# dguilliams3/book-recommendation-engine

Hardware: AMD Instinct MI355X
Metric: exact top-10 queries/sec at 10M×1536 fp32 (1/8 GPU) + % HBM/MFMA roofline (higher is better)
Workload: dtype fp32

## Files before the change

book-recommendation-engine_amd/csrc/vs_gemm_x1.hip:

```cpp
#include <algorithm>
#include <climits>
#include <cmath>
#include <cstdlib>
#include <type_traits>
#include <vector>

#include "vs_x1_device.h"

#ifndef VS_X1_PROBE
#define VS_X1_PROBE 0
#endif
#define VS_X1_P(bit) ((VS_X1_PROBE & (bit)) != 0)

namespace vs {

#ifndef VS_X1_STAMP
#define VS_X1_STAMP 0
#endif
constexpr int kStampSeg = 9;
constexpr int kStampCnt = 3;
constexpr int kStampHist = 16;
constexpr int kStampN = 2 * (kStampSeg + kStampCnt) + 2 + 2 * kStampHist;
__device__ unsigned long long g_x1_stamps[kStampN];

// ... 766 lines not shown
    auto seg_step = [&](auto first_tag) {
      constexpr bool first = decltype(first_tag)::value;
      __builtin_amdgcn_sched_barrier(0);
      if constexpr (S16) {
        rd16(buf);
      } else {
        rd(buf, 0, fa0, fb0);
        rd(buf, 1, fa1, fb1);
      }
      __builtin_amdgcn_sched_barrier(0);
      stage_step();
      advance_cursor();
      __builtin_amdgcn_sched_barrier(0);
      VS_X1_MARK(0);
      asm volatile("s_waitcnt vmcnt(8)" ::: "memory");
      VS_X1_MARK(1);
      __builtin_amdgcn_s_barrier();
      __builtin_amdgcn_sched_barrier(0);
      VS_X1_MARK(2);
      if constexpr (S16) {
#pragma unroll
        for (int b = 0; b < 8; ++b) mfma16_b(b, first_tag);
      } else {
        if constexpr (first) {
#pragma unroll
          for (int rb = 0; rb < 4; ++rb) mfma_rb_first(rb, fa0, fb0);
        } else {
#pragma unroll
          for (int rb = 0; rb < 4; ++rb) mfma_rb(rb, fa0, fb0);
        }
#pragma unroll
        for (int rb = 0; rb < 4; ++rb) mfma_rb(rb, fa1, fb1);
      }
      __builtin_amdgcn_sched_barrier(0);
      VS_X1_MARK(3);
      __builtin_amdgcn_s_barrier();
      __builtin_amdgcn_sched_barrier(0);
      VS_X1_MARK(4);
      VS_X1_MARK(5);
      buf = buf + 1 == NBUF ? 0 : buf + 1;
    };
    auto seg_tiles = [&]() {
      for (int t = t0; t < t1; ++t) {
        seg_step(std::true_type{});
        for (int k = 1; k < nksteps; ++k) seg_step(std::false_type{});
        if constexpr (!VS_X1_P(8)) {
          if constexpr (S16) epilogue16(t);
          else epilogue(t);
        } else if constexpr (S16) {
#pragma unroll
          for (int b = 0; b < 8; ++b)
#pragma unroll
            for (int qb = 0; qb < 4; ++qb) asm volatile("" ::"v"(acc16[b][qb]));
        } else {
#pragma unroll
          for (int rb = 0; rb < 4; ++rb)
#pragma unroll
            for (int qb = 0; qb < 2; ++qb) asm volatile("" ::"v"(acc[rb][qb]));
        }
        VS_X1_MARK(5);
      }
    };
    seg_tiles();
    if (!lag) __builtin_amdgcn_s_barrier();
#undef VS_X1_MARK
    }
#if VS_X1_STAMP
    {
      const int grp = w >= 4 ? 1 : 0;
      if (lane == 0) {
#pragma unroll
        for (int i = 0; i < kStampSeg; ++i)
          atomicAdd(&g_x1_stamps[grp * (kStampSeg + kStampCnt) + i], sg[i]);
        atomicAdd(&g_x1_stamps[2 * (kStampSeg + kStampCnt) + grp], (unsigned long long)nsteps);
      }
      if (lane == 0)
        atomicAdd(&g_x1_stamps[grp * (kStampSeg + kStampCnt) + kStampSeg], ecnt[0]);
      if constexpr (S16) {
        const int bin = nev < kStampHist ? nev : kStampHist - 1;
        for (int v = 0; v < kStampHist; ++v) {
          const unsigned long long m = __ballot(bin == v);
          if (lane == 0 && m)
            atomicAdd(&g_x1_stamps[2 * (kStampSeg + kStampCnt) + 2 + (chunk == 1 ? 0 : kStampHist) + v],
                      (unsigned long long)__popcll(m));
        }
      }
    }
#endif
    asm volatile("s_waitcnt vmcnt(0)" ::: "memory");
  }

  const int ln = (int)__builtin_amdgcn_mbcnt_hi(~0u, __builtin_amdgcn_mbcnt_lo(~0u, 0u));
  const int pl0 = sp * 4 + wr * 2 + (S16 ? (ln >> 4) & 1 : ln >> 5);
#pragma unroll
  for (int qb = 0; qb < NQB; ++qb) {
    const int64_t g =
        (int64_t)(qt * kT + 64 * wq + (S16 ? 16 * qb + (ln & 15) : 32 * qb + (ln & 31))) * P + pl0;
    if constexpr (VS_X1_P(256) && DUMP) {
      asm volatile("" ::"v"(dc[qb]), "v"(g));
    } else if constexpr (S16) {
      if (ln < 32) dcount[g] = dc[qb];
    } else if constexpr (DUMP) {
      dcount[g] = dc[qb];
    } else {
      const int64_t o = g * KP;
#pragma unroll
      for (int e = 0; e < KR; ++e) {
        pkey[o + e] = lk[qb][e];
        pid[o + e] = li[qb][e];
      }
      for (int e = KR; e < KP; ++e) {
        pkey[o + e] = FLT_MAX;
        pid[o + e] = -1;
      }
    }
  }
}

static int x1_qg() {
  static const int v = [] {
    const char* e = getenv("VS_X1_QG");
    const int q = e ? atoi(e) : 0;
    return q > 0 ? q : 4;
  }();
  return v;
}

static bool x1_group_rounds() {
  const char* e = getenv("VS_X1_XCDG");
  return !e || atoi(e) != 0;
}

constexpr int kX1SplitDen = 8;

constexpr int kX1ShortChunkTiles = 40;
static int x1_chunk_tiles(int per_block, bool can_dump) {
  const char* e = getenv("VS_X1_CHUNK_TILES");
  const int v = e ? atoi(e) : 0;
  if (v > 0) return v;
  return can_dump && per_block >= 128 && per_block <= 3 * kX1ChunkTiles ? kX1ShortChunkTiles
                                                                        : kX1ChunkTiles;
}

static int x1_split_den() {
  const char* e = getenv("VS_X1_SPLIT");
  return e ? std::max(0, atoi(e)) : kX1SplitDen;
}
constexpr int kSplitMinTiles = 16;
static int x1_first_den(int el, bool ecut) {
  const char* e = getenv("VS_X1_QUARTER");
  if (!e) return el == FILTER_BF16 || ecut ? 4 : 0;
  const int v = atoi(e);
  return v == 1 ? 4 : v >= 2 ? v : 0;
}

enum X1Kind : int { kX1List = 0, kX1Dump32 = 2, kX1Dump16 = 3 };
enum : int {
  kX1Replay = 1,
  kX1FirstCut = 2,
  kX1ReplayCut = 4,
  kX1ExactCut = 8,
};
struct X1Step {
  int p0, p1;
  int kind;
  int after;
};
struct X1Plan {
  int nparts = 1;
  bool cutting = false;
  std::vector<X1Step> step;
  int nlaunch() const { return (int)step.size(); }
};
static X1Plan x1_plan(int per_block, bool can_dump, int el, bool ecut, bool gathered, int recut) {
  X1Plan p;
  const bool dump = can_dump && !gathered;
  const int chunk_tiles = x1_chunk_tiles(per_block, dump);
  const int nchunk = gathered ? 1 : std::max(1, (per_block + chunk_tiles - 1) / chunk_tiles);
  const int den = x1_split_den();
  const bool split = dump && nchunk < 4 && den >= 2 && per_block >= kSplitMinTiles;
  p.cutting = dump && (nchunk >= 4 || split);
  const int F = x1_first_den(el, ecut);
  const bool quarter =
      p.cutting && !split && nchunk >= 4 && F >= 2 && per_block / (F * nchunk) >= 2;
  p.nparts = split ? den : quarter ? F * nchunk : nchunk;
  const int nlaunch = split ? 2 : quarter ? nchunk + 1 : nchunk;
  for (int c = 0; c < nlaunch; ++c) {
    X1Step s;
    s.p0 = split     ? (c == 0 ? 0 : 1)
           : quarter ? (c == 0 ? 0 : c == 1 ? 1 : F * (c - 1))
                     : c;
    s.p1 = split     ? (c == 0 ? 1 : den)
           : quarter ? (c == 0 ? 1 : F * c)
                     : c + 1;
    s.kind = p.cutting && c > 0 ? kX1Dump32 : kX1List;
    s.after = 0;
    if (p.cutting && c == 0) s.after |= kX1FirstCut | (ecut ? kX1ExactCut : 0);
    if (p.cutting && c > 0 && (((c + 1) & c) == 0 || c + 1 == nlaunch)) {
      const bool again = recut && c + 1 < nlaunch;
      s.after |= again ? kX1ReplayCut | (ecut ? kX1ExactCut : 0) : kX1Replay;
    }
    p.step.push_back(s);
  }
  return p;
}
static int x1_dump_kind(int mode, int el, bool dump32) {
  return x1_has_s16(mode, el) && !dump32 ? kX1Dump16 : kX1Dump32;
}

template <int KR, int MODE, int EL>
static hipError_t x1_launch(const X1Args& a, Partials part, hipStream_t st, int* ndispatch) {
  const int ntiles = (a.ntotal + kT - 1) / kT;
  const int nqt = a.nq_pad / kT;
  const int per_block = (ntiles + a.nsplit - 1) / a.nsplit;
  const int qg = a.qcount ? nqt : x1_qg() * (x1_group_rounds() ? 1 : -1);
  const bool dump = a.dump && x1_has_dump(MODE, EL) && !a.qcount && a.qcut && a.qbkey &&
                    a.qcut_m > 0 && a.dcount && a.dslot && a.dR > 0;
  const bool ecut = MODE == MODE_IP && EL == FILTER_I8 && a.ecut_x && a.qam;
  const X1Plan plan = x1_plan(per_block, dump, EL, ecut, a.qcount != nullptr, a.recut);
  const int nlaunch = plan.nlaunch();
  const int64_t ldb = a.ld * filter_bytes(EL);
  if (a.qtile0 < 0) return hipErrorInvalidValue;
  auto launch = [&](auto kernel, const X1Step& s, bool dumps) {
    hipLaunchKernelGGL(kernel, dim3(nqt * a.nsplit), dim3(512), 0, st, (const char*)a.XH, a.xs,
                       a.xaux, (const char*)a.QH, a.qs, a.qaux, a.nqa, (int)(ldb / 64), a.ntotal,
                       ntiles, a.nsplit, nqt, a.qtile0, a.self0, a.qrow, a.qcount, s.p0, s.p1,
                       plan.nparts, part.KP, qg, part.key, part.id, a.xgmax, a.xgmin,
                       dumps ? a.qcut : nullptr, dumps ? a.dcount : nullptr,
                       dumps ? a.dslot : nullptr, dumps ? a.dR : 0, a.qskip);
  };
  for (int c = 0; c < nlaunch; ++c) {
    const X1Step& s = plan.step[c];
    if (a.timing)
      a.timing->begin(st, !(plan.cutting && nlaunch > 1) || c > 0,
                      (double)(s.p1 - s.p0) / plan.nparts);
    switch (s.kind == kX1Dump32 ? x1_dump_kind(MODE, EL, a.dump32) : s.kind) {
      case kX1Dump16:
        if constexpr (x1_has_s16(MODE, EL))
          launch(gemm_topk_x1<KR, MODE, true, EL, true>, s, true);
        break;
      case kX1Dump32:
        if constexpr (x1_has_dump(MODE, EL)) launch(gemm_topk_x1<KR, MODE, true, EL>, s, true);
        break;
      default:
        launch(gemm_topk_x1<KR, MODE, false, EL>, s, false);
    }
    if (a.timing) a.timing->end(st);
    hipError_t e = hipGetLastError();
    if (e == hipSuccess && (s.after & kX1Replay)) e = launch_x1_replay(a, part, st);
    if (e == hipSuccess && (s.after & kX1FirstCut)) e = launch_qcut(a, part, st);
    if (e == hipSuccess && (s.after & kX1ReplayCut)) e = launch_x1_replay_cut(a, part, st);
    if (e == hipSuccess && (s.after & kX1ExactCut)) e = launch_x1_ecut(a, part, st);
    if (e != hipSuccess) return e;
  }
  if (ndispatch) *ndispatch = nlaunch;
  return hipSuccess;
}

int x1_lane_len() { return 8; }
int x1_dump_slots() { return kDumpMaxR; }
bool x1_pass_dumps(int ntotal, int nsplit) {
  const int ntiles = (ntotal + kT - 1) / kT;
  return x1_plan((ntiles + nsplit - 1) / nsplit, true, FILTER_I8, false, false, 1).cutting;
}

bool x1_plan_describe(int mode, int filter, int64_t ntotal, int nsplit, bool can_dump, bool ecut,
                      bool gathered, int recut, bool dump32, int32_t* out, int cap,
                      int* nlaunch) {
  if ((filter != FILTER_I8 && filter != FILTER_BF16) || ntotal <= 0 || ntotal > INT_MAX ||
      nsplit < 1 || (mode != MODE_IP && mode != MODE_L2 && mode != MODE_COS))
    return false;
  const int64_t ntiles = (ntotal + kT - 1) / kT;
  const X1Plan plan =
      x1_plan((int)((ntiles + nsplit - 1) / nsplit), can_dump && x1_has_dump(mode, filter), filter,
              ecut && mode == MODE_IP && filter == FILTER_I8, gathered, recut);
  out[0] = plan.nparts, out[1] = plan.cutting, out[2] = 0, out[3] = plan.cutting;
  out[4] = x1_pass_dumps((int)ntotal, nsplit);
  for (int c = 0; c < plan.nlaunch() && c < cap; ++c) {
    const X1Step& s = plan.step[c];
    int32_t* o = out + 5 + 4 * c;
    o[0] = s.p0, o[1] = s.p1, o[3] = s.after;
    o[2] = s.kind == kX1Dump32 ? x1_dump_kind(mode, filter, dump32) : s.kind;
  }
  *nlaunch = plan.nlaunch();
  return true;
}

hipError_t x1_stamps(unsigned long long* out, int reset) {
  hipError_t e = hipMemcpyFromSymbol(out, HIP_SYMBOL(g_x1_stamps), sizeof(g_x1_stamps));
  if (e == hipSuccess && reset) {
    unsigned long long z[kStampN] = {};
    e = hipMemcpyToSymbol(HIP_SYMBOL(g_x1_stamps), z, sizeof(z));
  }
  return e;
}

template <int EL>
static hipError_t x1_dispatch(int mode, const X1Args& a, Partials part, hipStream_t st,
                              int* ndispatch) {
  switch (mode) {
    case MODE_IP:
      return x1_launch<8, MODE_IP, EL>(a, part, st, ndispatch);
    case MODE_L2:
      if constexpr (EL == FILTER_I8) return hipErrorInvalidValue;
      else return x1_launch<8, MODE_L2, EL>(a, part, st, ndispatch);
    case MODE_COS:
      return x1_launch<8, MODE_COS, EL>(a, part, st, ndispatch);
    default:
      return hipErrorInvalidValue;
  }
}

hipError_t launch_gemm_topk_x1(int mode, const X1Args& a, Partials part, hipStream_t st,
                               int* ndispatch) {
  if (a.nq_pad % kT != 0 || a.ld % 64 != 0 || a.ld <= 0 || part.KP < x1_lane_len() ||
      part.P != 4 * a.nsplit || a.nsplit < 1 || a.ntotal <= 0)
    return hipErrorInvalidValue;
  if (a.filter == FILTER_I8) {
    if (!a.xs || !a.qs || !a.xgmax || !a.xgmin || a.ld > kI8MaxLd) return hipErrorInvalidValue;
    return x1_dispatch<FILTER_I8>(mode, a, part, st, ndispatch);
  }
  return x1_dispatch<FILTER_BF16>(mode, a, part, st, ndispatch);
}

bool x1_dump_applies(int mode, int filter) { return x1_has_dump(mode, filter); }

int x1_list_len(int need) {
  return need + 8 <= 24   ? 24
         : need + 8 <= 32 ? 32
         : need + 8 <= 64 ? 64
         : need < 128 ? 128
         : need < 256 ? 256
         : need < 512 ? 512
         : need < kVerifyMaxKF ? kVerifyMaxKF
                               : 0;
}

}
```

book-recommendation-engine_amd/csrc/vs_x1_cuts.hip:

```cpp
#include <algorithm>
#include <climits>
#include <cmath>
#include <cstdlib>

#include "vs_x1_device.h"

namespace vs {


template <int KR, int EL>
__global__ __launch_bounds__(256) void x1_replay_kernel(
    int* __restrict__ dcount, const int* __restrict__ dslot, float* __restrict__ pkey,
    int* __restrict__ pid, int P, int KP, int nqa, const float* __restrict__ qs,
    const float* __restrict__ xs, int64_t self0, int ntotal, int dR, int64_t nl,
    float* __restrict__ qcut, unsigned long long* __restrict__ stats) {
  const int64_t i = (int64_t)blockIdx.x * 256 + threadIdx.x;
  const int cnt = i < (int64_t)nqa * P ? dcount[i] : 0;
  replay_stats(cnt, dR, stats);
  if (cnt == 0) return;
  dcount[i] = 0;
  const int q = (int)(i / P);
  if (cnt > dR) {
    qcut[q] = -FLT_MAX;
    return;
  }
  const float cut = qcut[q];
  const float qsc = EL == FILTER_I8 ? qs[q] : 0.0f;
  const int selfrow = self0 >= 0 ? (int)(self0 + q) : -1;
  float lk[KR];
  int li[KR];
  const int64_t o = i * KP;
  lane_list_load<KR>(pkey, pid, o, lk, li);
  replay_admit<KR, EL>(lk, li, dslot, i, nl, cnt, qsc, xs, selfrow, ntotal, cut);
  lane_list_store<KR>(pkey, pid, o, lk, li);
}

hipError_t launch_x1_replay(const X1Args& a, Partials part, hipStream_t st) {
  unsigned long long* stats = a.dstats;
  if (!a.dump || !a.dcount || a.nqa <= 0) return hipSuccess;
  if (part.KP < x1_lane_len() || part.KP % 4 != 0) return hipErrorInvalidValue;
  const int64_t n = (int64_t)a.nqa * part.P;
  const dim3 grid((unsigned)((n + 255) / 256));
  const int64_t nl = (int64_t)a.nq_pad * part.P;
  if (a.filter == FILTER_I8)
    hipLaunchKernelGGL((x1_replay_kernel<8, FILTER_I8>), grid, dim3(256), 0, st, a.dcount, a.dslot,
                       part.key, part.id, part.P, part.KP, a.nqa, a.qs, a.xs, a.self0, a.ntotal,
                       a.dR, nl, a.qcut, stats);
  else
    hipLaunchKernelGGL((x1_replay_kernel<8, FILTER_BF16>), grid, dim3(256), 0, st, a.dcount,
                       a.dslot, part.key, part.id, part.P, part.KP, a.nqa, a.qs, a.xs, a.self0,
                       a.ntotal, a.dR, nl, a.qcut, stats);
  return hipGetLastError();
}

constexpr int kQcutThreads = 256;
__global__ __launch_bounds__(kQcutThreads) void qcut_kernel(
    const float* __restrict__ lkey, const int* __restrict__ lid, int P, int LKP, int L, int M,
    const double* __restrict__ bkey, int nq, float* __restrict__ cut, float* __restrict__ qam) {
  const int q = blockIdx.x;
  const int tid = threadIdx.x;
  if (q >= nq) return;
  const int64_t base = (int64_t)q * P * LKP;
  const int n = P * L;
  constexpr int kR = 16;
  uint64_t v[kR];
  const bool regs = n <= kQcutThreads * kR;
  auto image = [&](int j) -> uint64_t {
    const int64_t o = base + (int64_t)(j / L) * LKP + j % L;
    return lid[o] >= 0 ? (uint64_t)key_order(lkey[o]) : (1ull << 32);
  };
#pragma unroll
  for (int i = 0; i < kR; ++i) {
    const int j = tid + kQcutThreads * i;
    v[i] = regs && j < n ? image(j) : (1ull << 32);
  }
  __shared__ int part[kQcutThreads / 64];
  auto count_below = [&](uint64_t y) {
    int c = 0;
    if (regs) {
#pragma unroll
      for (int i = 0; i < kR; ++i) c += v[i] < y ? 1 : 0;
    } else {
      for (int j = tid; j < n; j += kQcutThreads) c += image(j) < y ? 1 : 0;
    }
    for (int o = 32; o > 0; o >>= 1) c += __shfl_xor(c, o);
    __syncthreads();
    if ((tid & 63) == 0) part[tid >> 6] = c;
    __syncthreads();
    int t = 0;
#pragma unroll
    for (int w = 0; w < kQcutThreads / 64; ++w) t += part[w];
    return t;
  };
  if (count_below(1ull << 32) < M) return;
  uint64_t x = 0;
  for (int b = 31; b >= 0; --b)
    if (count_below(x + (1ull << b)) < M) x += 1ull << b;
  const float aM = key_unorder((uint32_t)x);
  if (tid == 0 && qam) qam[q] = aM;
  if (tid == 0) {
    const float old = cut[q];
    const float t = lower_cut(aM, 2.000001, bkey[q], old);
    if (t < old) cut[q] = t;
  }
}

hipError_t launch_qcut(const X1Args& a, Partials part, hipStream_t st) {
  const int nq = a.nqa;
  hipLaunchKernelGGL(qcut_kernel, dim3(nq), dim3(kQcutThreads), 0, st, part.key, part.id, part.P, part.KP,
                     x1_lane_len(), a.qcut_m, a.qbkey, nq, a.qcut, a.qam);
  return hipGetLastError();
}

template <int KR, int EL>
__global__ __launch_bounds__(256) void x1_replay_cut_kernel(
    int* __restrict__ dcount, const int* __restrict__ dslot, float* __restrict__ pkey,
    int* __restrict__ pid, int P, int KP, const float* __restrict__ qs,
    const float* __restrict__ xs, int64_t self0, int ntotal, int dR, int64_t nl,
    float* __restrict__ qcut, unsigned long long* __restrict__ stats, int M,
    const double* __restrict__ bkey, float* __restrict__ qam) {
  __shared__ int hist[256];
  __shared__ int wsum[4];
  __shared__ int s_over, sel_digit, sel_before;
  const int q = blockIdx.x;
  const int tid = threadIdx.x, lane = tid & 63, wv = tid >> 6;
  const int nth = blockDim.x, nwv = nth >> 6;
  const bool has = tid < P;
  const int64_t i = (int64_t)q * P + tid;
  const int cnt = has ? dcount[i] : 0;
  replay_stats(cnt, dR, stats);
  if (tid == 0) s_over = 0;
  const float cut = qcut[q];
  float lk[KR];
  int li[KR];
  const int64_t o = i * KP;
#pragma unroll
  for (int e = 0; e < KR; ++e) lk[e] = FLT_MAX, li[e] = -1;
  if (has) lane_list_load<KR>(pkey, pid, o, lk, li);
  __syncthreads();
  if (cnt > 0) {
    dcount[i] = 0;
    if (cnt > dR) {
      s_over = 1;
    } else {
      const float qsc = EL == FILTER_I8 ? qs[q] : 0.0f;
      const int selfrow = self0 >= 0 ? (int)(self0 + q) : -1;
      replay_admit<KR, EL>(lk, li, dslot, i, nl, cnt, qsc, xs, selfrow, ntotal, cut);
      lane_list_store<KR>(pkey, pid, o, lk, li);
    }
  }
  __syncthreads();
  if (s_over) {
    if (tid == 0) qcut[q] = -FLT_MAX;
    return;
  }
  if (cut == -FLT_MAX) return;
  uint32_t v[KR];
  int nv = 0;
#pragma unroll
  for (int e = 0; e < KR; ++e) {
    v[e] = key_order(lk[e]);
    nv += li[e] >= 0 ? 1 : 0;
  }
  for (int o2 = 32; o2 > 0; o2 >>= 1) nv += __shfl_xor(nv, o2);
  if (lane == 0) wsum[wv] = nv;
  __syncthreads();
  int total = 0;
  for (int w2 = 0; w2 < nwv; ++w2) total += wsum[w2];
  if (total < M) return;
  uint32_t pre = 0;
  int want = M;
  for (int sh = 24; sh >= 0; sh -= 8) {
    for (int b = tid; b < 256; b += nth) hist[b] = 0;
    __syncthreads();
#pragma unroll
    for (int e = 0; e < KR; ++e)
      if (li[e] >= 0 && (sh == 24 || (v[e] >> (sh + 8)) == (pre >> (sh + 8))))
        atomicAdd(&hist[(v[e] >> sh) & 0xFF], 1);
    __syncthreads();
    if (wv == 0) {
      const int h0 = hist[4 * lane], h1 = hist[4 * lane + 1], h2 = hist[4 * lane + 2],
                h3 = hist[4 * lane + 3];
      const int own = h0 + h1 + h2 + h3;
      int inc = own;
      for (int o2 = 1; o2 < 64; o2 <<= 1) {
        const int t = __shfl_up(inc, o2);
        if (lane >= o2) inc += t;
      }
      const int before = inc - own;
      if (before < want && want <= inc) {
        int c = before, d = 4 * lane;
        const int hh[4] = {h0, h1, h2, h3};
        for (int e = 0; e < 4; ++e) {
          if (c + hh[e] >= want) {
            d = 4 * lane + e;
            break;
          }
          c += hh[e];
        }
        sel_digit = d;
        sel_before = c;
      }
    }
    __syncthreads();
    pre |= (uint32_t)sel_digit << sh;
    want -= sel_before;
  }
  if (tid == 0) {
    const float aM = key_unorder(pre);
    if (qam) qam[q] = aM;
    const float t = lower_cut(aM, 2.000001, bkey[q], cut);
    if (t < cut) qcut[q] = t;
  }
}

constexpr int kReplayCutMaxP = 256;

hipError_t launch_x1_replay_cut(const X1Args& a, Partials part, hipStream_t st) {
  if (!a.dump || !a.dcount || a.nqa <= 0) return hipSuccess;
  if (part.KP < x1_lane_len() || part.KP % 4 != 0) return hipErrorInvalidValue;
  if (a.recut == 2 || part.P > kReplayCutMaxP) {
    const hipError_t e = launch_x1_replay(a, part, st);
    return e != hipSuccess ? e : launch_qcut(a, part, st);
  }
  const int64_t nl = (int64_t)a.nq_pad * part.P;
  const dim3 block((unsigned)((part.P + 63) / 64 * 64));
  if (a.filter == FILTER_I8)
    hipLaunchKernelGGL((x1_replay_cut_kernel<8, FILTER_I8>), dim3(a.nqa), block, 0, st, a.dcount,
                       a.dslot, part.key, part.id, part.P, part.KP, a.qs, a.xs, a.self0, a.ntotal,
                       a.dR, nl, a.qcut, a.dstats, a.qcut_m, a.qbkey, a.qam);
  else
    hipLaunchKernelGGL((x1_replay_cut_kernel<8, FILTER_BF16>), dim3(a.nqa), block, 0, st, a.dcount,
                       a.dslot, part.key, part.id, part.P, part.KP, a.qs, a.xs, a.self0, a.ntotal,
                       a.dR, nl, a.qcut, a.dstats, a.qcut_m, a.qbkey, a.qam);
  return hipGetLastError();
}

constexpr int kEcutCand = 64;
__global__ __launch_bounds__(256) void x1_ecut_kernel(
    const float* __restrict__ lkey, const int* __restrict__ lid, int P, int LKP, int L, int M,
    const double* __restrict__ bkey, const float* __restrict__ qam, const float* __restrict__ X,
    const float* __restrict__ Q, int64_t ld, int ntotal, float* __restrict__ ckey,
    int* __restrict__ cid, float* __restrict__ qcut) {
  constexpr int kU = kEcutMaxM + kEcutCand;
  __shared__ int cand[kEcutCand];
  __shared__ float uk[kU];
  __shared__ int ui[kU];
  __shared__ int wsum[4];
  __shared__ int un;
  const int q = blockIdx.x;
  const int tid = threadIdx.x, lane = tid & 63, wv = tid >> 6;
  const float cut = qcut[q];
  const float aM = qam[q];
  float* ck = ckey + (int64_t)q * kEcutMaxM;
  int* ci = cid + (int64_t)q * kEcutMaxM;
  if (tid < kEcutMaxM) {
    ui[tid] = ci[tid];
    uk[tid] = ck[tid];
  }
  const float* qrow = Q + (int64_t)q * ld;
  const bool pairs = ld <= 256 * kQV;
  QSlice qsl;
  if (pairs) load_qslice(qrow, ld, lane, qsl);
  if (cut == -FLT_MAX || !(aM < FLT_MAX)) return;
  const bool vec = L == 8 && LKP % 4 == 0;
  int ncand = 0;
  for (int p0 = 0; p0 < P && ncand < kEcutCand; p0 += 256) {
    const int p = p0 + tid;
    int ids[8];
    float lk[8];
    int c = 0;
    const int64_t o = ((int64_t)q * P + p) * LKP;
#pragma unroll
    for (int e = 0; e < 8; ++e) ids[e] = -1, lk[e] = FLT_MAX;
    if (p < P && vec) {
#pragma unroll
      for (int e = 0; e < 8; e += 4) {
        const f32x4 kv = *(const f32x4*)(lkey + o + e);
        const int4 iv = *(const int4*)(lid + o + e);
        lk[e] = kv.x, lk[e + 1] = kv.y, lk[e + 2] = kv.z, lk[e + 3] = kv.w;
        ids[e] = iv.x, ids[e + 1] = iv.y, ids[e + 2] = iv.z, ids[e + 3] = iv.w;
      }
    } else if (p < P) {
#pragma unroll
      for (int e = 0; e < 8; ++e)
        if (e < L) ids[e] = lid[o + e], lk[e] = lkey[o + e];
    }
#pragma unroll
    for (int e = 0; e < 8; ++e) {
      if (ids[e] >= 0 && ids[e] < ntotal && lk[e] <= aM)
        ++c;
      else
        ids[e] = -1;
    }
    int inc = c;
    for (int o2 = 1; o2 < 64; o2 <<= 1) {
      const int t = __shfl_up(inc, o2);
      if (lane >= o2) inc += t;
    }
    __syncthreads();
    if (lane == 63) wsum[wv] = inc;
    __syncthreads();
    int before = ncand + inc - c;
    for (int w = 0; w < wv; ++w) before += wsum[w];
#pragma unroll
    for (int e = 0; e < 8; ++e)
      if (ids[e] >= 0) {
        if (before < kEcutCand) cand[before] = ids[e];
        ++before;
      }
    ncand += wsum[0] + wsum[1] + wsum[2] + wsum[3];
  }
  ncand = min(ncand, kEcutCand);
  __syncthreads();
  int m0 = 0;
  for (int t = 0; t < kEcutMaxM; ++t) m0 += ui[t] >= 0 ? 1 : 0;
  if (tid == 0) un = m0;
  __syncthreads();
  if (tid < ncand) {
    const int r = cand[tid];
    bool found = false;
    for (int t = 0; t < m0; ++t) found |= ui[t] == r;
    if (!found) ui[atomicAdd(&un, 1)] = r;
  }
  __syncthreads();
  const int n = un;
  if (pairs) {
    for (int j = m0 + 2 * wv; j < n; j += 8) {
      const int ra = ui[j], rb = j + 1 < n ? ui[j + 1] : ra;
      double da, db;
      wave_dot2<false, float>(X + (int64_t)ra * ld, X + (int64_t)rb * ld, qsl, ld, lane, da, db);
      if (lane == 0) {
        uk[j] = exact_key<MODE_IP>((float)da, q, ra, nullptr, nullptr, nullptr, nullptr);
        if (j + 1 < n)
          uk[j + 1] = exact_key<MODE_IP>((float)db, q, rb, nullptr, nullptr, nullptr, nullptr);
      }
    }
  } else {
    for (int j = m0 + wv; j < n; j += 4) {
      const int r = ui[j];
      const double acc = wave_dot<false, float>(X + (int64_t)r * ld, qrow, ld, lane);
      if (lane == 0) uk[j] = exact_key<MODE_IP>((float)acc, q, r, nullptr, nullptr, nullptr, nullptr);
    }
  }
  __syncthreads();
  if (tid < n) {
    const float k0 = uk[tid];
    const int i0 = ui[tid];
    int rank = 0;
    for (int t = 0; t < n; ++t) rank += lex_less(uk[t], ui[t], k0, i0) ? 1 : 0;
    if (rank < M) {
      ck[rank] = k0;
      ci[rank] = i0;
    }
    if (rank == M - 1) {
      const float t = lower_cut(k0, 1.000001, bkey[q], cut);
      if (t < cut) qcut[q] = t;
    }
  }
}

hipError_t launch_x1_ecut(const X1Args& a, Partials part, hipStream_t st) {
  if (!a.ecut_x || !a.ecut_q || !a.qam || !a.ecut_key || !a.ecut_id || a.nqa <= 0)
    return hipSuccess;
  if (a.qcut_m < 1 || a.qcut_m > kEcutMaxM || a.ecut_ld % 4 != 0 || x1_lane_len() > 8)
    return hipErrorInvalidValue;
  hipLaunchKernelGGL(x1_ecut_kernel, dim3(a.nqa), dim3(256), 0, st, part.key, part.id, part.P,
                     part.KP, x1_lane_len(), a.qcut_m, a.qbkey, a.qam, a.ecut_x, a.ecut_q,
                     a.ecut_ld, a.ntotal, a.ecut_key, a.ecut_id, a.qcut);
  return hipGetLastError();
}

}
```

book-recommendation-engine_amd/csrc/vs_x1_device.h:

```cpp
#pragma once

#include "vs_device.h"

namespace vs {

__device__ __forceinline__ f32x4 row4(const float* __restrict__ p) { return *(const f32x4*)p; }
__device__ __forceinline__ f32x4 row4(const uint16_t* __restrict__ p) {
  const uint2 u = *(const uint2*)p;
  return f32x4{__uint_as_float(u.x << 16), __uint_as_float(u.x & 0xFFFF0000u),
               __uint_as_float(u.y << 16), __uint_as_float(u.y & 0xFFFF0000u)};
}

template <int EL>
__device__ __forceinline__ float x1_key(int sum_bits, float qsc, float fx) {
  if constexpr (EL == FILTER_I8) return -((float)sum_bits * (qsc * fx));
  else return -__int_as_float(sum_bits);
}

__device__ __forceinline__ uint32_t key_order(float f) {
  const uint32_t u = __float_as_uint(f);
  return (u & 0x80000000u) ? ~u : (u | 0x80000000u);
}
__device__ __forceinline__ float key_unorder(uint32_t u) {
  return __uint_as_float((u & 0x80000000u) ? (u & 0x7FFFFFFFu) : ~u);
// ... 2 lines not shown
template <bool DIFF = false, typename RT = float>
__device__ __forceinline__ double wave_dot(const RT* __restrict__ x, const float* __restrict__ q,
                                           int64_t ld, int lane) {
  double acc = 0.0;
  for (int64_t c = lane * 4; c < ld; c += 256) {
    const f32x4 xv = row4(x + c);
    const f32x4 qv = *(const f32x4*)(q + c);
#pragma unroll
    for (int e = 0; e < 4; ++e) {
      if constexpr (DIFF) {
        const double t = (double)xv[e] - (double)qv[e];
        acc = fma(t, t, acc);
      } else {
        acc = fma((double)xv[e], (double)qv[e], acc);
      }
    }
  }
  for (int o = 32; o > 0; o >>= 1) acc += __shfl_xor(acc, o);
  return acc;
}

constexpr int kQV = 8;
struct QSlice {
  f32x4 v[kQV];
};
__device__ __forceinline__ void load_qslice(const float* __restrict__ q, int64_t ld, int lane,
                                            QSlice& qs) {
#pragma unroll
  for (int i = 0; i < kQV; ++i) {
    const int64_t c = lane * 4 + 256 * i;
    qs.v[i] = c < ld ? *(const f32x4*)(q + c) : f32x4{0.f, 0.f, 0.f, 0.f};
  }
}
template <bool DIFF = false, typename RT = float>
__device__ __forceinline__ void wave_dot2(const RT* __restrict__ xa, const RT* __restrict__ xb,
                                          const QSlice& qs, int64_t ld, int lane, double& ra,
                                          double& rb) {
  f32x4 va[kQV], vb[kQV];
#pragma unroll
  for (int i = 0; i < kQV; ++i) {
    const int64_t c = lane * 4 + 256 * i;
    va[i] = c < ld ? row4(xa + c) : f32x4{0.f, 0.f, 0.f, 0.f};
    vb[i] = c < ld ? row4(xb + c) : f32x4{0.f, 0.f, 0.f, 0.f};
  }
  double a = 0.0, b = 0.0;
#pragma unroll
  for (int i = 0; i < kQV; ++i) {
    if (lane * 4 + 256 * i >= ld) break;
#pragma unroll
    for (int e = 0; e < 4; ++e) {
      if constexpr (DIFF) {
        const double ta = (double)va[i][e] - (double)qs.v[i][e];
        const double tb = (double)vb[i][e] - (double)qs.v[i][e];
        a = fma(ta, ta, a);
        b = fma(tb, tb, b);
      } else {
        a = fma((double)va[i][e], (double)qs.v[i][e], a);
        b = fma((double)vb[i][e], (double)qs.v[i][e], b);
      }
    }
  }
  for (int o = 32; o > 0; o >>= 1) {
    a += __shfl_xor(a, o);
    b += __shfl_xor(b, o);
  }
  ra = a;
  rb = b;
}

template <int MODE>
__device__ __forceinline__ float exact_key(float ip, int q, int r, const float* __restrict__ qn,
                                           const float* __restrict__ xn,
                                           const float* __restrict__ qinv,
                                           const float* __restrict__ xinv) {
  return MODE == MODE_L2    ? l2_from_ip(qn[q], xn[r], ip)
         : MODE == MODE_COS ? -(ip * (qinv[q] * xinv[r]))
         : MODE == MODE_L2D ? ip
                            : -ip;
}


__device__ __forceinline__ void replay_stats(int cnt, int dR,
                                             unsigned long long* __restrict__ stats) {
  unsigned long long a = (unsigned long long)cnt, b = cnt > dR ? 1ull : 0ull;
  for (int o = 32; o > 0; o >>= 1) {
    a += __shfl_xor(a, o);
    b += __shfl_xor(b, o);
  }
  if ((threadIdx.x & 63) == 0 && a && stats) {
    atomicAdd(stats, a);
    if (b) atomicAdd(stats + 1, b);
  }
}

template <int KR>
__device__ __forceinline__ void lane_list_load(const float* __restrict__ pkey,
                                               const int* __restrict__ pid, int64_t o,
                                               float (&lk)[KR], int (&li)[KR]) {
  static_assert(KR % 4 == 0, "lane lists move as 16-B pieces");
#pragma unroll
  for (int e = 0; e < KR; e += 4) {
    const f32x4 kv = *(const f32x4*)(pkey + o + e);
    const int4 iv = *(const int4*)(pid + o + e);
    lk[e] = kv.x, lk[e + 1] = kv.y, lk[e + 2] = kv.z, lk[e + 3] = kv.w;
    li[e] = iv.x, li[e + 1] = iv.y, li[e + 2] = iv.z, li[e + 3] = iv.w;
  }
}
template <int KR>
__device__ __forceinline__ void lane_list_store(float* __restrict__ pkey, int* __restrict__ pid,
                                                int64_t o, const float (&lk)[KR],
                                                const int (&li)[KR]) {
#pragma unroll
  for (int e = 0; e < KR; e += 4) {
    *(f32x4*)(pkey + o + e) = f32x4{lk[e], lk[e + 1], lk[e + 2], lk[e + 3]};
    *(int4*)(pid + o + e) = make_int4(li[e], li[e + 1], li[e + 2], li[e + 3]);
  }
}

template <int KR, int EL>
__device__ __forceinline__ void replay_admit(float (&lk)[KR], int (&li)[KR],
                                             const int* __restrict__ dslot, int64_t i, int64_t nl,
                                             int cnt, float qsc, const float* __restrict__ xs,
                                             int selfrow, int ntotal, float cut) {
  const i32x2* sl = (const i32x2*)dslot + i;
  constexpr int kB = 8;
  for (int c0 = 0; c0 < cnt; c0 += kB) {
    i32x2 e[kB];
    float fx[kB];
#pragma unroll
    for (int j = 0; j < kB; ++j) e[j] = c0 + j < cnt ? sl[(int64_t)(c0 + j) * nl] : i32x2{-1, 0};
#pragma unroll
    for (int j = 0; j < kB; ++j)
      fx[j] = EL == FILTER_I8 && e[j][0] >= 0 && e[j][0] < ntotal ? xs[e[j][0]] : 0.0f;
#pragma unroll
    for (int j = 0; j < kB; ++j) {
      const int row = e[j][0];
      if (!(row >= 0 && row < ntotal && row != selfrow)) continue;
      const float key = x1_key<EL>(e[j][1], qsc, fx[j]);
      if (key < fminf(lk[KR - 1], cut)) list_insert<KR, int>(lk, li, key, row);
    }
  }
}

__device__ __forceinline__ float lower_cut(float base, double factor, double B, float old) {
  const double tp = (double)base + factor * B;
  if (isfinite(tp) && tp < (double)FLT_MAX) {
    float t = (float)tp;
    if ((double)t < tp) t = nextafterf(t, INFINITY);
    if (t < old) return t;
  }
  return old;
}

hipError_t launch_qcut(const X1Args& a, Partials part, hipStream_t st);
hipError_t launch_x1_replay_cut(const X1Args& a, Partials part, hipStream_t st);
hipError_t launch_x1_ecut(const X1Args& a, Partials part, hipStream_t st);

}
```

Before: 90550.

## Fuse exact-cut refresh into qcut and replay-cut kernels, share radix select

Moves the exact-cut refresh logic into a shared device function and calls it at the end of the qcut and replay-cut kernels, so the separate ecut kernel launch and its reload of the lane lists are avoided. The replay-cut path passes its register-held lists straight in. qcut swaps its 32-step bitwise binary search for the radix select already used by replay-cut, and cut kernels now use 128 threads by default. An opt-in env flag merges consecutive dump launches. This adds shared-memory pressure and a smaller block, which can slow the exact dot products.

```diff
diff --git a/book-recommendation-engine_amd/csrc/vs_gemm_x1.hip b/book-recommendation-engine_amd/csrc/vs_gemm_x1.hip
--- a/book-recommendation-engine_amd/csrc/vs_gemm_x1.hip
+++ b/book-recommendation-engine_amd/csrc/vs_gemm_x1.hip
@@ -942,6 +942,11 @@
   if (!e) return el == FILTER_BF16 || ecut ? 4 : 0;
   const int v = atoi(e);
   return v == 1 ? 4 : v >= 2 ? v : 0;
+}
+
+static bool x1_merge() {
+  const char* e = getenv("VS_X1_MERGE");
+  return e && atoi(e) != 0;
 }
 
 enum X1Kind : int { kX1List = 0, kX1Dump32 = 2, kX1Dump16 = 3 };
@@ -990,7 +995,13 @@
       const bool again = recut && c + 1 < nlaunch;
       s.after |= again ? kX1ReplayCut | (ecut ? kX1ExactCut : 0) : kX1Replay;
     }
-    p.step.push_back(s);
+    if (x1_merge() && s.kind == kX1Dump32 && !p.step.empty() &&
+        p.step.back().kind == kX1Dump32 && p.step.back().after == 0) {
+      p.step.back().p1 = s.p1;
+      p.step.back().after = s.after;
+    } else {
+      p.step.push_back(s);
+    }
   }
   return p;
 }
@@ -1038,9 +1049,9 @@
     if (a.timing) a.timing->end(st);
     hipError_t e = hipGetLastError();
     if (e == hipSuccess && (s.after & kX1Replay)) e = launch_x1_replay(a, part, st);
-    if (e == hipSuccess && (s.after & kX1FirstCut)) e = launch_qcut(a, part, st);
-    if (e == hipSuccess && (s.after & kX1ReplayCut)) e = launch_x1_replay_cut(a, part, st);
-    if (e == hipSuccess && (s.after & kX1ExactCut)) e = launch_x1_ecut(a, part, st);
+    const bool ex = (s.after & kX1ExactCut) != 0;
+    if (e == hipSuccess && (s.after & kX1FirstCut)) e = launch_qcut(a, part, st, ex);
+    if (e == hipSuccess && (s.after & kX1ReplayCut)) e = launch_x1_replay_cut(a, part, st, ex);
     if (e != hipSuccess) return e;
   }
   if (ndispatch) *ndispatch = nlaunch;
diff --git a/book-recommendation-engine_amd/csrc/vs_x1_cuts.hip b/book-recommendation-engine_amd/csrc/vs_x1_cuts.hip
--- a/book-recommendation-engine_amd/csrc/vs_x1_cuts.hip
+++ b/book-recommendation-engine_amd/csrc/vs_x1_cuts.hip
@@ -53,10 +53,213 @@
   return hipGetLastError();
 }
 
-constexpr int kQcutThreads = 256;
+constexpr int kEcutCand = 64;
+#ifndef VS_X1_CUT_THREADS
+#define VS_X1_CUT_THREADS 128
+#endif
+constexpr int kCutThreads = VS_X1_CUT_THREADS;
+constexpr int kReplayCutMaxP = 256;
+static_assert(kCutThreads % 64 == 0 && kCutThreads >= kEcutMaxM + kEcutCand &&
+                  kCutThreads <= kReplayCutMaxP,
+              "ecut_refresh");
+struct EcutArgs {
+  const float* X = nullptr;
+  const float* Q = nullptr;
+  int64_t ld = 0;
+  float* ckey = nullptr;
+  int* cid = nullptr;
+};
+struct EcutShared {
+  int cand[kEcutCand];
+  float uk[kEcutMaxM + kEcutCand];
+  int ui[kEcutMaxM + kEcutCand];
+  int wsum[kReplayCutMaxP / 64];
+  int un;
+};
+template <bool HELD>
+__device__ __forceinline__ void ecut_refresh(EcutShared& sh, int q, const float* __restrict__ lkey,
+                                             const int* __restrict__ lid, int P, int LKP, int L,
+                                             int M, const double* __restrict__ bkey, float aM,
+                                             float cut, float stored, const EcutArgs& ec,
+                                             int ntotal, float* __restrict__ qcut,
+                                             const float (&hk)[8], const int (&hi)[8]) {
+  const int nth = blockDim.x, kW = nth >> 6;
+  int* cand = sh.cand;
+  float* uk = sh.uk;
+  int* ui = sh.ui;
+  int* wsum = sh.wsum;
+  const int tid = threadIdx.x, lane = tid & 63, wv = tid >> 6;
+  const int64_t ld = ec.ld;
+  float* ck = ec.ckey + (int64_t)q * kEcutMaxM;
+  int* ci = ec.cid + (int64_t)q * kEcutMaxM;
+  if (tid < kEcutMaxM) {
+    ui[tid] = ci[tid];
+    uk[tid] = ck[tid];
+  }
+  const float* qrow = ec.Q + (int64_t)q * ld;
+  const bool pairs = ld <= 256 * kQV;
+  QSlice qsl;
+  if (pairs) load_qslice(qrow, ld, lane, qsl);
+  const bool vec = L == 8 && LKP % 4 == 0;
+  int ncand = 0;
+  for (int p0 = 0; p0 < P && ncand < kEcutCand; p0 += nth) {
+    const int p = p0 + tid;
+    int ids[8];
+    float lk[8];
+    int c = 0;
+    const int64_t o = ((int64_t)q * P + p) * LKP;
+#pragma unroll
+    for (int e = 0; e < 8; ++e) ids[e] = -1, lk[e] = FLT_MAX;
+    if constexpr (HELD) {
+      if (p < P) {
+#pragma unroll
+        for (int e = 0; e < 8; ++e) ids[e] = hi[e], lk[e] = hk[e];
+      }
+    } else if (p < P && vec) {
+#pragma unroll
+      for (int e = 0; e < 8; e += 4) {
+        const f32x4 kv = *(const f32x4*)(lkey + o + e);
+        const int4 iv = *(const int4*)(lid + o + e);
+        lk[e] = kv.x, lk[e + 1] = kv.y, lk[e + 2] = kv.z, lk[e + 3] = kv.w;
+        ids[e] = iv.x, ids[e + 1] = iv.y, ids[e + 2] = iv.z, ids[e + 3] = iv.w;
+      }
+    } else if (p < P) {
+#pragma unroll
+      for (int e = 0; e < 8; ++e)
+        if (e < L) ids[e] = lid[o + e], lk[e] = lkey[o + e];
+    }
+#pragma unroll
+    for (int e = 0; e < 8; ++e) {
+      if (ids[e] >= 0 && ids[e] < ntotal && lk[e] <= aM)
+        ++c;
+      else
+        ids[e] = -1;
+    }
+    int inc = c;
+    for (int o2 = 1; o2 < 64; o2 <<= 1) {
+      const int t = __shfl_up(inc, o2);
+      if (lane >= o2) inc += t;
+    }
+    __syncthreads();
+    if (lane == 63) wsum[wv] = inc;
+    __syncthreads();
+    int before = ncand + inc - c;
+    for (int w = 0; w < wv; ++w) before += wsum[w];
+#pragma unroll
+    for (int e = 0; e < 8; ++e)
+      if (ids[e] >= 0) {
+        if (before < kEcutCand) cand[before] = ids[e];
+        ++before;
+      }
+    for (int w = 0; w < kW; ++w) ncand += wsum[w];
+  }
+  ncand = min(ncand, kEcutCand);
+  __syncthreads();
+  int m0 = 0;
+  for (int t = 0; t < kEcutMaxM; ++t) m0 += ui[t] >= 0 ? 1 : 0;
+  if (tid == 0) sh.un = m0;
+  __syncthreads();
+  if (tid < ncand) {
+    const int r = cand[tid];
+    bool found = false;
+    for (int t = 0; t < m0; ++t) found |= ui[t] == r;
+    if (!found) ui[atomicAdd(&sh.un, 1)] = r;
+  }
+  __syncthreads();
+  const int n = sh.un;
+  if (pairs) {
+    for (int j = m0 + 2 * wv; j < n; j += 2 * kW) {
+      const int ra = ui[j], rb = j + 1 < n ? ui[j + 1] : ra;
+      double da, db;
+      wave_dot2<false, float>(ec.X + (int64_t)ra * ld, ec.X + (int64_t)rb * ld, qsl, ld, lane, da,
+                              db);
+      if (lane == 0) {
+        uk[j] = exact_key<MODE_IP>((float)da, q, ra, nullptr, nullptr, nullptr, nullptr);
+        if (j + 1 < n)
+          uk[j + 1] = exact_key<MODE_IP>((float)db, q, rb, nullptr, nullptr, nullptr, nullptr);
+      }
+    }
+  } else {
+    for (int j = m0 + wv; j < n; j += kW) {
+      const int r = ui[j];
+      const double acc = wave_dot<false, float>(ec.X + (int64_t)r * ld, qrow, ld, lane);
+      if (lane == 0) uk[j] = exact_key<MODE_IP>((float)acc, q, r, nullptr, nullptr, nullptr, nullptr);
+    }
+  }
+  __syncthreads();
+  if (tid < n) {
+    const float k0 = uk[tid];
+    const int i0 = ui[tid];
+    int rank = 0;
+    for (int t = 0; t < n; ++t) rank += lex_less(uk[t], ui[t], k0, i0) ? 1 : 0;
+    if (rank < M) {
+      ck[rank] = k0;
+      ci[rank] = i0;
+    }
+    if (rank == M - 1) {
+      const float t = lower_cut(k0, 1.000001, bkey[q], cut);
+      if (t < stored) qcut[q] = t;
+    }
+  }
+  if (n < M && tid == 0 && cut < stored) qcut[q] = cut;
+}
+
+struct SelectShared {
+  int hist[256];
+  int digit, before;
+};
+template <int KV>
+__device__ __forceinline__ uint32_t select_mth(SelectShared& ss, const uint32_t (&v)[KV],
+                                               unsigned ok, int M) {
+  const int tid = threadIdx.x, lane = tid & 63, wv = tid >> 6, nth = blockDim.x;
+  uint32_t pre = 0;
+  int want = M;
+  for (int sh = 24; sh >= 0; sh -= 8) {
+    for (int b = tid; b < 256; b += nth) ss.hist[b] = 0;
+    __syncthreads();
+#pragma unroll
+    for (int e = 0; e < KV; ++e)
+      if (((ok >> e) & 1u) && (sh == 24 || (v[e] >> (sh + 8)) == (pre >> (sh + 8))))
+        atomicAdd(&ss.hist[(v[e] >> sh) & 0xFF], 1);
+    __syncthreads();
+    if (wv == 0) {
+      const int h0 = ss.hist[4 * lane], h1 = ss.hist[4 * lane + 1], h2 = ss.hist[4 * lane + 2],
+                h3 = ss.hist[4 * lane + 3];
+      const int own = h0 + h1 + h2 + h3;
+      int inc = own;
+      for (int o2 = 1; o2 < 64; o2 <<= 1) {
+        const int t = __shfl_up(inc, o2);
+        if (lane >= o2) inc += t;
+      }
+      const int before = inc - own;
+      if (before < want && want <= inc) {
+        int c = before, d = 4 * lane;
+        const int hh[4] = {h0, h1, h2, h3};
+        for (int e = 0; e < 4; ++e) {
+          if (c + hh[e] >= want) {
+            d = 4 * lane + e;
+            break;
+          }
+          c += hh[e];
+        }
+        ss.digit = d;
+        ss.before = c;
+      }
+    }
+    __syncthreads();
+    pre |= (uint32_t)ss.digit << sh;
+    want -= ss.before;
+  }
+  return pre;
+}
+
+constexpr int kQcutThreads = kCutThreads;
 __global__ __launch_bounds__(kQcutThreads) void qcut_kernel(
     const float* __restrict__ lkey, const int* __restrict__ lid, int P, int LKP, int L, int M,
-    const double* __restrict__ bkey, int nq, float* __restrict__ cut, float* __restrict__ qam) {
+    const double* __restrict__ bkey, int nq, float* __restrict__ cut, float* __restrict__ qam,
+    EcutArgs ec, int ntotal) {
+  __shared__ EcutShared esh;
+  __shared__ SelectShared ssh;
   const int q = blockIdx.x;
   const int tid = threadIdx.x;
   if (q >= nq) return;
@@ -94,34 +297,65 @@
   };
   if (count_below(1ull << 32) < M) return;
   uint64_t x = 0;
-  for (int b = 31; b >= 0; --b)
-    if (count_below(x + (1ull << b)) < M) x += 1ull << b;
+  if (regs) {
+    uint32_t v32[kR];
+    unsigned ok = 0;
+#pragma unroll
+    for (int i = 0; i < kR; ++i) {
+      v32[i] = (uint32_t)v[i];
+      ok |= v[i] < (1ull << 32) ? 1u << i : 0u;
+    }
+    x = select_mth<kR>(ssh, v32, ok, M);
+  } else {
+    for (int b = 31; b >= 0; --b)
+      if (count_below(x + (1ull << b)) < M) x += 1ull << b;
+  }
   const float aM = key_unorder((uint32_t)x);
   if (tid == 0 && qam) qam[q] = aM;
-  if (tid == 0) {
-    const float old = cut[q];
-    const float t = lower_cut(aM, 2.000001, bkey[q], old);
-    if (t < old) cut[q] = t;
-  }
-}
-
-hipError_t launch_qcut(const X1Args& a, Partials part, hipStream_t st) {
+  const float old = cut[q];
+  const float t = lower_cut(aM, 2.000001, bkey[q], old);
+  if (ec.X && t != -FLT_MAX) {
+    const float none_k[8] = {};
+    const int none_i[8] = {};
+    ecut_refresh<false>(esh, q, lkey, lid, P, LKP, L, M, bkey, aM, t, old, ec, ntotal, cut, none_k,
+                        none_i);
+  } else if (tid == 0 && t < old) {
+    cut[q] = t;
+  }
+}
+
+static hipError_t ecut_args(const X1Args& a, bool want, EcutArgs* ec) {
+  *ec = EcutArgs{};
+  if (!want || !a.ecut_x || !a.ecut_q || !a.qam || !a.ecut_key || !a.ecut_id) return hipSuccess;
+  if (a.qcut_m < 1 || a.qcut_m > kEcutMaxM || a.ecut_ld % 4 != 0 || x1_lane_len() > 8)
+    return hipErrorInvalidValue;
+  ec->X = a.ecut_x, ec->Q = a.ecut_q, ec->ld = a.ecut_ld, ec->ckey = a.ecut_key, ec->cid = a.ecut_id;
+  return hipSuccess;
+}
+
+hipError_t launch_qcut(const X1Args& a, Partials part, hipStream_t st, bool ecut) {
   const int nq = a.nqa;
+  EcutArgs ec;
+  const hipError_t e0 = ecut_args(a, ecut && a.recut != 2, &ec);
+  if (e0 != hipSuccess) return e0;
   hipLaunchKernelGGL(qcut_kernel, dim3(nq), dim3(kQcutThreads), 0, st, part.key, part.id, part.P, part.KP,
-                     x1_lane_len(), a.qcut_m, a.qbkey, nq, a.qcut, a.qam);
-  return hipGetLastError();
+                     x1_lane_len(), a.qcut_m, a.qbkey, nq, a.qcut, a.qam, ec, a.ntotal);
+  const hipError_t e = hipGetLastError();
+  return e == hipSuccess && ecut && a.recut == 2 ? launch_x1_ecut(a, part, st) : e;
 }
 
 template <int KR, int EL>
-__global__ __launch_bounds__(256) void x1_replay_cut_kernel(
+__global__ __launch_bounds__(kReplayCutMaxP) void x1_replay_cut_kernel(
     int* __restrict__ dcount, const int* __restrict__ dslot, float* __restrict__ pkey,
     int* __restrict__ pid, int P, int KP, const float* __restrict__ qs,
     const float* __restrict__ xs, int64_t self0, int ntotal, int dR, int64_t nl,
     float* __restrict__ qcut, unsigned long long* __restrict__ stats, int M,
-    const double* __restrict__ bkey, float* __restrict__ qam) {
-  __shared__ int hist[256];
-  __shared__ int wsum[4];
-  __shared__ int s_over, sel_digit, sel_before;
+    const double* __restrict__ bkey, float* __restrict__ qam, EcutArgs ec) {
+  static_assert(KR == 8, "ecut_refresh takes lane lists of 8");
+  __shared__ SelectShared ssh;
+  __shared__ int wsum[kReplayCutMaxP / 64];
+  __shared__ EcutShared esh;
+  __shared__ int s_over;
   const int q = blockIdx.x;
   const int tid = threadIdx.x, lane = tid & 63, wv = tid >> 6;
   const int nth = blockDim.x, nwv = nth >> 6;
@@ -168,206 +402,66 @@
   int total = 0;
   for (int w2 = 0; w2 < nwv; ++w2) total += wsum[w2];
   if (total < M) return;
-  uint32_t pre = 0;
-  int want = M;
-  for (int sh = 24; sh >= 0; sh -= 8) {
-    for (int b = tid; b < 256; b += nth) hist[b] = 0;
-    __syncthreads();
-#pragma unroll
-    for (int e = 0; e < KR; ++e)
-      if (li[e] >= 0 && (sh == 24 || (v[e] >> (sh + 8)) == (pre >> (sh + 8))))
-        atomicAdd(&hist[(v[e] >> sh) & 0xFF], 1);
-    __syncthreads();
-    if (wv == 0) {
-      const int h0 = hist[4 * lane], h1 = hist[4 * lane + 1], h2 = hist[4 * lane + 2],
-                h3 = hist[4 * lane + 3];
-      const int own = h0 + h1 + h2 + h3;
-      int inc = own;
-      for (int o2 = 1; o2 < 64; o2 <<= 1) {
-        const int t = __shfl_up(inc, o2);
-        if (lane >= o2) inc += t;
-      }
-      const int before = inc - own;
-      if (before < want && want <= inc) {
-        int c = before, d = 4 * lane;
-        const int hh[4] = {h0, h1, h2, h3};
-        for (int e = 0; e < 4; ++e) {
-          if (c + hh[e] >= want) {
-            d = 4 * lane + e;
-            break;
-          }
-          c += hh[e];
-        }
-        sel_digit = d;
-        sel_before = c;
-      }
-    }
-    __syncthreads();
-    pre |= (uint32_t)sel_digit << sh;
-    want -= sel_before;
-  }
-  if (tid == 0) {
-    const float aM = key_unorder(pre);
-    if (qam) qam[q] = aM;
-    const float t = lower_cut(aM, 2.000001, bkey[q], cut);
-    if (t < cut) qcut[q] = t;
-  }
-}
-
-constexpr int kReplayCutMaxP = 256;
-
-hipError_t launch_x1_replay_cut(const X1Args& a, Partials part, hipStream_t st) {
-  if (!a.dump || !a.dcount || a.nqa <= 0) return hipSuccess;
+  unsigned ok = 0;
+#pragma unroll
+  for (int e = 0; e < KR; ++e) ok |= li[e] >= 0 ? 1u << e : 0u;
+  const uint32_t pre = select_mth<KR>(ssh, v, ok, M);
+  const float aM = key_unorder(pre);
+  if (tid == 0 && qam) qam[q] = aM;
+  const float t = lower_cut(aM, 2.000001, bkey[q], cut);
+  if (ec.X && t != -FLT_MAX) {
+    ecut_refresh<true>(esh, q, pkey, pid, P, KP, KR, M, bkey, aM, t, cut, ec, ntotal, qcut, lk, li);
+  } else if (tid == 0 && t < cut) {
+    qcut[q] = t;
+  }
+}
+
+
+hipError_t launch_x1_replay_cut(const X1Args& a, Partials part, hipStream_t st, bool ecut) {
+  if (!a.dump || !a.dcount || a.nqa <= 0)
+    return ecut && a.recut == 2 ? launch_x1_ecut(a, part, st) : hipSuccess;
   if (part.KP < x1_lane_len() || part.KP % 4 != 0) return hipErrorInvalidValue;
   if (a.recut == 2 || part.P > kReplayCutMaxP) {
     const hipError_t e = launch_x1_replay(a, part, st);
-    return e != hipSuccess ? e : launch_qcut(a, part, st);
-  }
+    return e != hipSuccess ? e : launch_qcut(a, part, st, ecut);
+  }
+  EcutArgs ec;
+  const hipError_t e0 = ecut_args(a, ecut, &ec);
+  if (e0 != hipSuccess) return e0;
   const int64_t nl = (int64_t)a.nq_pad * part.P;
-  const dim3 block((unsigned)((part.P + 63) / 64 * 64));
+  const dim3 block((unsigned)std::max(kCutThreads, (part.P + 63) / 64 * 64));
   if (a.filter == FILTER_I8)
     hipLaunchKernelGGL((x1_replay_cut_kernel<8, FILTER_I8>), dim3(a.nqa), block, 0, st, a.dcount,
                        a.dslot, part.key, part.id, part.P, part.KP, a.qs, a.xs, a.self0, a.ntotal,
-                       a.dR, nl, a.qcut, a.dstats, a.qcut_m, a.qbkey, a.qam);
+                       a.dR, nl, a.qcut, a.dstats, a.qcut_m, a.qbkey, a.qam, ec);
   else
     hipLaunchKernelGGL((x1_replay_cut_kernel<8, FILTER_BF16>), dim3(a.nqa), block, 0, st, a.dcount,
                        a.dslot, part.key, part.id, part.P, part.KP, a.qs, a.xs, a.self0, a.ntotal,
-                       a.dR, nl, a.qcut, a.dstats, a.qcut_m, a.qbkey, a.qam);
+                       a.dR, nl, a.qcut, a.dstats, a.qcut_m, a.qbkey, a.qam, ec);
   return hipGetLastError();
 }
 
-constexpr int kEcutCand = 64;
-__global__ __launch_bounds__(256) void x1_ecut_kernel(
+__global__ __launch_bounds__(kCutThreads) void x1_ecut_kernel(
     const float* __restrict__ lkey, const int* __restrict__ lid, int P, int LKP, int L, int M,
-    const double* __restrict__ bkey, const float* __restrict__ qam, const float* __restrict__ X,
-    const float* __restrict__ Q, int64_t ld, int ntotal, float* __restrict__ ckey,
-    int* __restrict__ cid, float* __restrict__ qcut) {
-  constexpr int kU = kEcutMaxM + kEcutCand;
-  __shared__ int cand[kEcutCand];
-  __shared__ float uk[kU];
-  __shared__ int ui[kU];
-  __shared__ int wsum[4];
-  __shared__ int un;
+    const double* __restrict__ bkey, const float* __restrict__ qam, EcutArgs ec, int ntotal,
+    float* __restrict__ qcut) {
+  __shared__ EcutShared esh;
   const int q = blockIdx.x;
-  const int tid = threadIdx.x, lane = tid & 63, wv = tid >> 6;
   const float cut = qcut[q];
   const float aM = qam[q];
-  float* ck = ckey + (int64_t)q * kEcutMaxM;
-  int* ci = cid + (int64_t)q * kEcutMaxM;
-  if (tid < kEcutMaxM) {
-    ui[tid] = ci[tid];
-    uk[tid] = ck[tid];
-  }
-  const float* qrow = Q + (int64_t)q * ld;
-  const bool pairs = ld <= 256 * kQV;
-  QSlice qsl;
-  if (pairs) load_qslice(qrow, ld, lane, qsl);
   if (cut == -FLT_MAX || !(aM < FLT_MAX)) return;
-  const bool vec = L == 8 && LKP % 4 == 0;
-  int ncand = 0;
-  for (int p0 = 0; p0 < P && ncand < kEcutCand; p0 += 256) {
-    const int p = p0 + tid;
-    int ids[8];
-    float lk[8];
-    int c = 0;
-    const int64_t o = ((int64_t)q * P + p) * LKP;
-#pragma unroll
-    for (int e = 0; e < 8; ++e) ids[e] = -1, lk[e] = FLT_MAX;
-    if (p < P && vec) {
-#pragma unroll
-      for (int e = 0; e < 8; e += 4) {
-        const f32x4 kv = *(const f32x4*)(lkey + o + e);
-        const int4 iv = *(const int4*)(lid + o + e);
-        lk[e] = kv.x, lk[e + 1] = kv.y, lk[e + 2] = kv.z, lk[e + 3] = kv.w;
-        ids[e] = iv.x, ids[e + 1] = iv.y, ids[e + 2] = iv.z, ids[e + 3] = iv.w;
-      }
-    } else if (p < P) {
-#pragma unroll
-      for (int e = 0; e < 8; ++e)
-        if (e < L) ids[e] = lid[o + e], lk[e] = lkey[o + e];
-    }
-#pragma unroll
-    for (int e = 0; e < 8; ++e) {
-      if (ids[e] >= 0 && ids[e] < ntotal && lk[e] <= aM)
-        ++c;
-      else
-        ids[e] = -1;
-    }
-    int inc = c;
-    for (int o2 = 1; o2 < 64; o2 <<= 1) {
-      const int t = __shfl_up(inc, o2);
-      if (lane >= o2) inc += t;
-    }
-    __syncthreads();
-    if (lane == 63) wsum[wv] = inc;
-    __syncthreads();
-    int before = ncand + inc - c;
-    for (int w = 0; w < wv; ++w) before += wsum[w];
-#pragma unroll
-    for (int e = 0; e < 8; ++e)
-      if (ids[e] >= 0) {
-        if (before < kEcutCand) cand[before] = ids[e];
-        ++before;
-      }
-    ncand += wsum[0] + wsum[1] + wsum[2] + wsum[3];
-  }
-  ncand = min(ncand, kEcutCand);
-  __syncthreads();
-  int m0 = 0;
-  for (int t = 0; t < kEcutMaxM; ++t) m0 += ui[t] >= 0 ? 1 : 0;
-  if (tid == 0) un = m0;
-  __syncthreads();
-  if (tid < ncand) {
-    const int r = cand[tid];
-    bool found = false;
-    for (int t = 0; t < m0; ++t) found |= ui[t] == r;
-    if (!found) ui[atomicAdd(&un, 1)] = r;
-  }
-  __syncthreads();
-  const int n = un;
-  if (pairs) {
-    for (int j = m0 + 2 * wv; j < n; j += 8) {
-      const int ra = ui[j], rb = j + 1 < n ? ui[j + 1] : ra;
-      double da, db;
-      wave_dot2<false, float>(X + (int64_t)ra * ld, X + (int64_t)rb * ld, qsl, ld, lane, da, db);
-      if (lane == 0) {
-        uk[j] = exact_key<MODE_IP>((float)da, q, ra, nullptr, nullptr, nullptr, nullptr);
-        if (j + 1 < n)
-          uk[j + 1] = exact_key<MODE_IP>((float)db, q, rb, nullptr, nullptr, nullptr, nullptr);
-      }
-    }
-  } else {
-    for (int j = m0 + wv; j < n; j += 4) {
-      const int r = ui[j];
-      const double acc = wave_dot<false, float>(X + (int64_t)r * ld, qrow, ld, lane);
-      if (lane == 0) uk[j] = exact_key<MODE_IP>((float)acc, q, r, nullptr, nullptr, nullptr, nullptr);
-    }
-  }
-  __syncthreads();
-  if (tid < n) {
-    const float k0 = uk[tid];
-    const int i0 = ui[tid];
-    int rank = 0;
-    for (int t = 0; t < n; ++t) rank += lex_less(uk[t], ui[t], k0, i0) ? 1 : 0;
-    if (rank < M) {
-      ck[rank] = k0;
-      ci[rank] = i0;
-    }
-    if (rank == M - 1) {
-      const float t = lower_cut(k0, 1.000001, bkey[q], cut);
-      if (t < cut) qcut[q] = t;
-    }
-  }
+  const float none_k[8] = {};
+  const int none_i[8] = {};
+  ecut_refresh<false>(esh, q, lkey, lid, P, LKP, L, M, bkey, aM, cut, cut, ec, ntotal, qcut, none_k,
+                      none_i);
 }
 
 hipError_t launch_x1_ecut(const X1Args& a, Partials part, hipStream_t st) {
-  if (!a.ecut_x || !a.ecut_q || !a.qam || !a.ecut_key || !a.ecut_id || a.nqa <= 0)
-    return hipSuccess;
-  if (a.qcut_m < 1 || a.qcut_m > kEcutMaxM || a.ecut_ld % 4 != 0 || x1_lane_len() > 8)
-    return hipErrorInvalidValue;
-  hipLaunchKernelGGL(x1_ecut_kernel, dim3(a.nqa), dim3(256), 0, st, part.key, part.id, part.P,
-                     part.KP, x1_lane_len(), a.qcut_m, a.qbkey, a.qam, a.ecut_x, a.ecut_q,
-                     a.ecut_ld, a.ntotal, a.ecut_key, a.ecut_id, a.qcut);
+  EcutArgs ec;
+  const hipError_t e0 = ecut_args(a, true, &ec);
+  if (e0 != hipSuccess || !ec.X || a.nqa <= 0) return e0;
+  hipLaunchKernelGGL(x1_ecut_kernel, dim3(a.nqa), dim3(kCutThreads), 0, st, part.key, part.id,
+                     part.P, part.KP, x1_lane_len(), a.qcut_m, a.qbkey, a.qam, ec, a.ntotal, a.qcut);
   return hipGetLastError();
 }
 
diff --git a/book-recommendation-engine_amd/csrc/vs_x1_device.h b/book-recommendation-engine_amd/csrc/vs_x1_device.h
--- a/book-recommendation-engine_amd/csrc/vs_x1_device.h
+++ b/book-recommendation-engine_amd/csrc/vs_x1_device.h
@@ -178,8 +178,8 @@
   return old;
 }
 
-hipError_t launch_qcut(const X1Args& a, Partials part, hipStream_t st);
-hipError_t launch_x1_replay_cut(const X1Args& a, Partials part, hipStream_t st);
+hipError_t launch_qcut(const X1Args& a, Partials part, hipStream_t st, bool ecut);
+hipError_t launch_x1_replay_cut(const X1Args& a, Partials part, hipStream_t st, bool ecut);
 hipError_t launch_x1_ecut(const X1Args& a, Partials part, hipStream_t st);
 
 }
```

Result: no change. 91010 (median of 6 runs) (+0.5%).
